# jctemp/owl-path-tracer

Hardware: AMD Instinct MI355X
Metric: Msamples/sec at 1920x1080x1024spp (higher is better)
Workload: dtype f32; 1 GPU; C4 dragon.json on the 871400-triangle stand-in (dragon.obj.scene is a missing blob), 1920x1080, 1024 spp, max_path_depth 16, environment intensity 0, areaLight emission 30; triangles=871404, bvh_nodes=276150, bvh_depth=24

## Files before the change

### owl-path-tracer_amd/csrc/pt_api.cpp

```cpp
#include <hip/hip_runtime.h>

#include <algorithm>
#include <atomic>
#include <chrono>
#include <cmath>
#include <cstdarg>
#include <cstdio>
#include <cstring>
#include <string>
#include <thread>
#include <vector>

#include "pt_internal.h"
#include "pt_launch.h"
#include "pt_tiers.h"

static inline void pt_collapse_sliver(float* p)
{
    const double e1[3] = {(double)p[3] - (double)p[0], (double)p[4] - (double)p[1], (double)p[5] - (double)p[2]};
    const double e2[3] = {(double)p[6] - (double)p[0], (double)p[7] - (double)p[1], (double)p[8] - (double)p[2]};
    const double e3[3] = {(double)p[6] - (double)p[3], (double)p[7] - (double)p[4], (double)p[8] - (double)p[5]};
    const double n[3] = {e1[1] * e2[2] - e1[2] * e2[1], e1[2] * e2[0] - e1[0] * e2[2], e1[0] * e2[1] - e1[1] * e2[0]};
    const double n2 = n[0] * n[0] + n[1] * n[1] + n[2] * n[2];
    const double l1 = e1[0] * e1[0] + e1[1] * e1[1] + e1[2] * e1[2], l2 = e2[0] * e2[0] + e2[1] * e2[1] + e2[2] * e2[2], l3 = e3[0] * e3[0] + e3[1] * e3[1] + e3[2] * e3[2];
    const double L2 = l1 > l2 ? (l1 > l3 ? l1 : l3) : (l2 > l3 ? l2 : l3);
    if (!(n2 > 1e-10 * L2 * L2)) {
        for (int k = 3; k < 9; ++k) p[k] = p[k % 3];
    }
}
#define PT_AUTO_PLOC_TRIS 64000000

namespace {
std::string g_create_error;
}

namespace pti {

int fail(pt_ctx* c, int code, const char* fmt, ...)
{
    char buf[1024];
    va_list ap;
    va_start(ap, fmt);
    vsnprintf(buf, sizeof(buf), fmt, ap);
    va_end(ap);
    if (c) c->err = buf;
    else g_create_error = buf;
    return code;
}

int ensure(pt_ctx* c, DevBuf& b, size_t bytes)
{
    if (bytes == 0) bytes = 16;
    if (b.cap >= bytes) return PT_OK;
    if (b.p) HIP_TRY(c, hipFree(b.p));
    b.p = nullptr;
    b.cap = 0;
    HIP_TRY(c, hipMalloc(&b.p, bytes));
    b.cap = bytes;
    return PT_OK;
}

}
using pti::ensure;
using pti::fail;

namespace {

int upload(pt_ctx* c, DevBuf& b, const void* src, size_t bytes)
{
    int rc = ensure(c, b, bytes);
    if (rc) return rc;
    if (bytes) HIP_TRY(c, hipMemcpyAsync(b.p, src, bytes, hipMemcpyHostToDevice, c->stream));
    return PT_OK;
}

void release(DevBuf& b)
{
    if (b.p) (void)hipFree(b.p);
    b.p = nullptr;
    b.cap = 0;
}

void copy_env(pt_ctx* c, const pt_env* env)
{
    c->env = *env;
    c->env_map.w = c->env_map.h = 0;
    c->env_map.px.clear();
    if (env->map.width > 0 && env->map.height > 0 && env->map.rgba8) {
        c->env_map.w = env->map.width;
        c->env_map.h = env->map.height;
        c->env_map.px.assign(env->map.rgba8, env->map.rgba8 + (size_t)env->map.width * env->map.height);
    }
    c->env.map.rgba8 = nullptr;
}

int upload_env(pt_ctx* c)
{
    if (c->host_only) return PT_OK;
    if (c->env_map.w > 0) return upload(c, c->d_env, c->env_map.px.data(), c->env_map.px.size() * 4);
    return PT_OK;
}

int upload_materials(pt_ctx* c)
{
    if (c->host_only) return PT_OK;
    return upload(c, c->d_materials, c->materials.data(), c->materials.size() * sizeof(float));
}

void pack_materials(pt_ctx* c, const float* materials, int n)
{
// ... 525 lines not shown

void walk_params(pt_ctx* c, const pt_camera* cam, PtKernelParams& P)
{
    fill_params(c, P);
    {
        const float reach = c->bvh.pad * 4194304.0f;
        float far_o = 0.0f;
        for (int a = 0; a < 3; ++a) far_o = std::max(far_o, std::fabs(cam->origin[a]));
        P.box_exact = (c->box_exact > 0 || (c->box_exact < 0 && !(far_o <= reach))) ? 1 : 0;
    }
    if (c->kernel == 2 && c->quad && !c->nodes4.empty()) {
        P.nodes4 = (const PtNode4*)c->d_nodes4.p;
        P.root = c->root4;
        P.stack_entries = 3 * c->depth4 + 1;
    }
    if (c->kernel == 2 && c->groups && !c->nodes8.empty()) {
        P.nodes8 = (const PtNode8*)c->d_nodes8.p;
        P.root8 = c->root8;
        P.groups = c->groups;
    }
}

struct FramePlan {
    int variant = 0, use_count = 0;
    PtGeometry geo{};
    int bpc = 0, grid = 0;
    int ring_grid = 0;
    bool sorted = false;
    bool tiers = false;
    int pre = 0;
    int n_launch = 1, S = 0;
    Schedule sc;
    int tail_min = 16;
    uint32_t n_express = 0;
    int express_waves = 0, ns_express = 0;
};

int plan_chunks(pt_ctx* c, bool group_walk, int max_samples, FramePlan& f)
{
    f.tail_min = c->chunk_tail_min >= 0 ? c->chunk_tail_min : 16;
    f.S = max_samples;
    f.n_launch = f.sorted ? 2 : 1;
    const int ns = f.geo.ns;
    if (f.sorted) {
        const int rest = max_samples - f.pre;
        int sticky = c->sticky_pct;
        if (sticky < 1) {
            const double ratio = (double)c->n_pixels / ((double)c->num_cus * (double)f.bpc * (double)ns);
            sticky = (int)std::min(80.0, 50.0 + 6.0 * ratio);
        }
        if (c->chunk_tail_min < 0) f.tail_min = std::max(16, rest / 8);
        const int big = std::max(1, (int)((int64_t)rest * sticky / 100));
        f.sc = make_schedule(rest, big, rest - big, f.tail_min);
    } else {
        const int chunk = std::min(c->spp_per_launch > 0 ? c->spp_per_launch : c->chunk_spp, std::min(max_samples, 65535));
        f.sc = make_schedule(max_samples, chunk, 1, f.tail_min);
    }
    const int n_chunks = f.sc.n_chunks;
    if ((uint64_t)c->n_pixels * (uint64_t)n_chunks >= 0xfff00000ull) return fail(c, PT_E_LIMIT, "too many (pixel, chunk) tickets");
    if (n_chunks > 255 || c->n_pixels >= (1u << 24)) return fail(c, PT_E_LIMIT, "the wavefront kernel needs n_chunks <= 255 and < 2^24 pixels per rank (raise chunk_spp)");
    if (f.sorted && group_walk && n_chunks <= 254 && (uint64_t)c->n_pixels * (uint64_t)n_chunks < 0xE0000000ull) {
        int& rgrid = f.tiers ? f.ring_grid : f.grid;
        const double ratio = (double)c->n_pixels / ((double)rgrid * (double)ns);
        double permille = c->express_permille >= 0 ? (double)c->express_permille : (ratio <= 1.5 ? 10.0 : (ratio >= 4.0 ? 0.0 : 10.0 * (4.0 - ratio) / 2.5));
        const int nse = std::max(1, std::min(c->ns_express, ns));
        uint64_t want = (uint64_t)((double)c->n_pixels * permille / 1000.0);
        const int capacity = c->num_cus * f.bpc;
        const int cap_waves = std::max(rgrid / 8, std::min(capacity / 2, capacity - rgrid));
        want = std::min<uint64_t>(want, (uint64_t)cap_waves * (uint64_t)nse);
        if (want > 0 && want < c->n_pixels) {
            f.n_express = (uint32_t)want;
            f.express_waves = (int)((want + (uint64_t)nse - 1) / (uint64_t)nse);
            f.ns_express = nse;
            rgrid = std::min(capacity, (int)(((long)c->n_pixels - (long)f.n_express + ns - 1) / ns) + f.express_waves);
        }
    }
    return PT_OK;
}

int plan_frame(pt_ctx* c, const PtKernelParams& P, int max_samples, FramePlan& f)
{
    f.use_count = (c->count || (c->kernel == 2 && !P.nodes4)) ? 1 : 0;
    f.variant = c->kernel == 2 && c->fallback && !f.use_count ? 3 : c->kernel;
    const int group_entries = P.nodes8 ? 7 * c->depth8 + 1 : 0;
    int want_ns = c->slots_per_wave > 0 ? c->slots_per_wave : PT_DEFAULT_NS;
    const PtGeometry& g = f.geo;
    auto geometry = [&] { return pt_kernel_geometry(f.variant, f.use_count, P.stack_entries, group_entries, want_ns, P.box_exact, &f.geo); };
    hipError_t ge = geometry();
    if (ge == hipErrorInvalidConfiguration && f.variant == 2 && !f.use_count) {
        f.variant = 3;
        ge = geometry();
    }
    if (ge == hipErrorInvalidConfiguration)
        return fail(c, PT_E_LIMIT, f.use_count ? "the instrumented instance of the render kernel needs scratch in this build; such builds rendered wrong pixels and are refused (pt_kernel.hip; tests/test_abi_host.py reads hipcc's resource report)"
                                               : "this build of the render kernel spills registers to scratch even in its fallback instance; such builds rendered wrong pixels and are refused (pt_kernel.hip)");
    HIP_TRY(c, ge);
    if (c->kernel == 2 && c->slots_per_wave == 0 && g.max_blocks_per_cu > 0) {
        const long fit = (long)c->n_pixels / ((long)c->num_cus * 8);
        if (fit < want_ns) {
            want_ns = (int)std::max(64L, fit);
            HIP_TRY(c, geometry());
        }
    }
    if (g.max_blocks_per_cu < 1) return fail(c, PT_E_LIMIT, "render kernel does not fit a CU (LDS %zu bytes, BVH depth %d)", g.lds_bytes, c->bvh.depth);
    f.bpc = c->blocks_per_cu > 0 ? std::min(c->blocks_per_cu, g.max_blocks_per_cu) : g.max_blocks_per_cu;
    const long capacity = (long)c->num_cus * f.bpc;
    const int per_wg = c->kernel == 1 ? g.block : g.ns;
    f.grid = (int)std::max(1L, std::min(((long)c->n_pixels + per_wg - 1) / per_wg, capacity));
    f.pre = c->prepass_spp > 0 ? c->prepass_spp : 8;
    f.sorted = c->kernel == 2 && c->schedule == 1 && c->spp_per_launch == 0 && max_samples >= 4 * f.pre && max_samples <= 65535;
    if (f.sorted && P.nodes8 && c->whole != 0 && c->slots_per_wave == 0) {
        for (int nsd = 96; nsd <= 104 && !f.tiers; nsd += 8) {
            if (c->whole < 1 && (long)c->n_pixels + (long)PT_MAX_TIERS * nsd > capacity * nsd) continue;
            want_ns = nsd;
            HIP_TRY(c, geometry());
            if (g.max_blocks_per_cu >= f.bpc && g.ns == nsd) {
                f.tiers = true;
                f.ring_grid = (int)std::max(1L, std::min(((long)c->n_pixels + g.ns - 1) / g.ns, capacity));
                f.grid = (int)capacity;
            }
        }
        if (!f.tiers) {
            want_ns = PT_DEFAULT_NS;
            HIP_TRY(c, geometry());
        }
    }
    if (f.tiers && c->prepass_spp == 0 && max_samples >= 4 * 16) f.pre = 16;
    if (c->kernel == 1) {
        f.S = std::min(c->spp_per_launch > 0 ? std::min(c->spp_per_launch, max_samples) : max_samples, 65535);
        f.n_launch = (max_samples + f.S - 1) / f.S;
        return PT_OK;
    }
    return plan_chunks(c, P.nodes8 != nullptr, max_samples, f);
}

int frame_buffers(pt_ctx* c, const FramePlan& f, int W, int H, void* d_out_rgb, void* d_out_rgba8, hipStream_t stream)
{
    int rc;
    const int n_chunks = f.sc.n_chunks;
    if (f.geo.state_words && (rc = ensure(c, c->d_slots, f.geo.state_words * 4 * (size_t)f.grid))) return rc;
    if (f.sorted) {
        if ((rc = ensure(c, c->d_cost, (size_t)W * H))) return rc;
        if ((rc = ensure(c, c->d_bucket, (size_t)c->n_pixels))) return rc;
        HIP_TRY(c, hipMemsetAsync(c->d_cost.p, 0, (size_t)W * H, stream));
        if ((rc = ensure(c, c->d_sorted, (size_t)c->n_pixels * 4))) return rc;
        if ((rc = ensure(c, c->d_sort_scratch, pt_sort_scratch_bytes(c->n_pixels)))) return rc;
    }
    if (c->kernel == 2) {
        c->lap_ticks_ofs = ((256 + (size_t)(n_chunks + 3) * 4 + 255) / 256) * 256;
        const size_t laps_bytes = c->lap_ticks_ofs + ((size_t)PT_LAP_REGION(n_chunks) + (size_t)PT_LAP_REGION(1)) * 8;
        if ((rc = ensure(c, c->d_laps, laps_bytes))) return rc;
        if ((rc = ensure(c, c->d_ring, (size_t)c->n_pixels * 4 * (size_t)n_chunks))) return rc;
        HIP_TRY(c, hipMemsetAsync(c->d_laps.p, 0, laps_bytes, stream));
        if (n_chunks > 1) HIP_TRY(c, hipMemsetAsync(c->d_ring.p, 0, (size_t)c->n_pixels * 4 * (size_t)n_chunks, stream));
        if ((rc = ensure(c, c->d_params, sizeof(PtKernelParams) * (size_t)f.n_launch))) return rc;
    }
    c->last_chunks = n_chunks;
    if ((rc = ensure(c, c->d_heads, (size_t)f.n_launch * PT_HEADS_WORDS * 4))) return rc;
    HIP_TRY(c, hipMemsetAsync(c->d_heads.p, 0, (size_t)f.n_launch * PT_HEADS_WORDS * 4, stream));
    if (f.tiers && (rc = ensure(c, c->d_tiers, (1 + PT_MAX_TIERS * PT_TIER_WORDS) * 4))) return rc;
    HIP_TRY(c, hipMemsetAsync(d_out_rgb, 0, (size_t)W * H * 3 * sizeof(float), stream));
    if (d_out_rgba8) HIP_TRY(c, hipMemsetAsync(d_out_rgba8, 0, (size_t)W * H * 4, stream));
    if (f.n_launch > 1 || n_chunks > 1) {
        if ((rc = ensure(c, c->d_rng, (size_t)W * H * 4))) return rc;
        if ((rc = ensure(c, c->d_accum, (size_t)W * H * 12))) return rc;
    }
// ... 185 lines not shown
    if (!c || !out) return PT_E_INVALID;
    if (!c->host_only && c->ev_pending) {
        HIP_TRY(c, hipSetDevice(c->device));
        HIP_TRY(c, hipEventSynchronize(c->ev1));
        int wrc = check_watchdog(c);
        if (wrc) return wrc;
        float ms = 0.0f;
        HIP_TRY(c, hipEventElapsedTime(&ms, c->ev0, c->ev1));
        c->stats.kernel_ms = ms;
        c->stats.prepass_ms = 0.0;
        if (c->last_sorted) {
            HIP_TRY(c, hipEventElapsedTime(&ms, c->ev0, c->evm));
            c->stats.prepass_ms = ms;
        }
        c->stats.launches = c->last_launches;
        c->ev_pending = false;
        if (c->count && c->d_counters.p) {
            PtCounters h;
            HIP_TRY(c, hipMemcpy(&h, c->d_counters.p, sizeof(h), hipMemcpyDeviceToHost));
            c->stats.samples = h.samples; c->stats.rays = h.rays; c->stats.nodes = h.nodes; c->stats.tris = h.tris;
            c->stats.scatters = h.scatters; c->stats.env_misses = h.env_misses; c->stats.nan_retries = h.nan_retries;
            for (int i = 0; i < 32; ++i) c->stats.sched[i] = h.sched[i];
            for (int i = 0; i < 8; ++i) c->stats.groups[i] = h.grp[i];
            for (int i = 0; i < 16; ++i) c->stats.lobes[i] = h.lobes[i];
            for (int i = 0; i < 4; ++i) c->stats.trav[i] = h.trav[i];
        }
    }
    *out = c->stats;
    return PT_OK;
}

void pt_to_camera_data(const float look_from[3], const float look_at[3], const float look_up[3], float vfov, int32_t w, int32_t h, pt_camera* out)
{
    auto dot = [](const float* a, const float* b) { return std::fma(a[2], b[2], std::fma(a[1], b[1], a[0] * b[0])); };
    auto cross = [](const float* a, const float* b, float* r) {
        r[0] = std::fma(a[1], b[2], -(a[2] * b[1]));
        r[1] = std::fma(a[2], b[0], -(a[0] * b[2]));
        r[2] = std::fma(a[0], b[1], -(a[1] * b[0]));
    };
    auto normalize = [&](float* v) {
        float s = 1.0f / std::sqrt(dot(v, v));
        v[0] *= s; v[1] *= s; v[2] *= s;
    };
    const float pi = 3.14159265358979323f;
    float aspect = (float)w / (float)h;
    float theta = vfov * pi / 180.0f;
    float hh = std::tan(theta / 2);
    float vh = 2.0f * hh, vw = aspect * vh;
    float W[3] = {look_from[0] - look_at[0], look_from[1] - look_at[1], look_from[2] - look_at[2]};
    normalize(W);
    float U[3], Vv[3];
    cross(look_up, W, U);
    normalize(U);
    cross(W, U, Vv);
    normalize(Vv);
    for (int i = 0; i < 3; ++i) {
        out->origin[i] = look_from[i];
        out->horizontal[i] = vw * U[i];
        out->vertical[i] = vh * Vv[i];
        out->llc[i] = look_from[i] - out->horizontal[i] / 2.0f - out->vertical[i] / 2.0f - W[i];
    }
}

int pt_debug_closest_hit_host(pt_ctx* c, const float org[3], const float dir[3], float tmin, float tmax, float* t, float* u, float* v, int32_t* prim)
{
    if (!c || !c->have_scene) return PT_E_NO_SCENE;
    return pt_bvh_closest_hit_host(c->bvh, org, dir, tmin, tmax, t, u, v, prim) ? 1 : 0;
}

int pt_debug_clone_scene(pt_ctx* dst, const pt_ctx* src)
{
    if (!dst || !src || dst == src) return PT_E_INVALID;
    return pti::clone_scene(dst, src);
}

int pt_debug_quad_info(pt_ctx* c, int64_t out[8])
{
    if (!c || !out) return PT_E_INVALID;
    if (!c->have_scene) return fail(c, PT_E_NO_SCENE, "pt_debug_quad_info before pt_upload_scene");
    int64_t leaf_slots = 0, tris = 0, empty = 0, internal = 0, bin_leaves = 0;
    for (const PtNode4& q : c->nodes4) {
        for (int k = 0; k < 4; ++k) {
            const int32_t r = q.child[k];
            if (r >= 0) ++internal;
            else if (r == -1) {
                ++empty;
                for (int a = 0; a < 3; ++a)
                    if (!(q.lo[a][k] == INFINITY && q.hi[a][k] == INFINITY)) return fail(c, PT_E_LIMIT, "quad node: empty slot with a finite box");
            } else {
                ++leaf_slots;
                tris += (int64_t)(~(uint32_t)r & 7u);
            }
        }
    }
    for (const PtNode& nd : c->bvh.nodes) {
        if (nd.left < -1) ++bin_leaves;
        if (nd.right < -1) ++bin_leaves;
    }
    out[0] = (int64_t)c->nodes4.size(); out[1] = c->depth4; out[2] = leaf_slots; out[3] = tris; out[4] = empty; out[5] = internal;
    out[6] = (int64_t)c->bvh.nodes.size(); out[7] = bin_leaves;
    return PT_OK;
}

int pt_debug_oct_info(pt_ctx* c, int64_t out[8])
{
    if (!c || !out) return PT_E_INVALID;
    if (!c->have_scene) return fail(c, PT_E_NO_SCENE, "pt_debug_oct_info before pt_upload_scene");
    int64_t leaf_slots = 0, tris = 0, empty = 0, internal = 0, max_leaf = 0;
    std::vector<uint8_t> seen(c->bvh.tris.size(), 0);
    std::vector<uint8_t> referenced(c->nodes8.size(), 0);
    for (const PtNode8& q : c->nodes8) {
        for (int k = 0; k < 8; ++k) {
            const int32_t r = q.c[k].ref;
            if (r >= 0) {
                if ((size_t)r >= c->nodes8.size() || referenced[(size_t)r]++) return fail(c, PT_E_LIMIT, "oct node: child %d out of range or referenced twice", r);
                ++internal;
            } else if (r == -1) {
                ++empty;
                for (int a = 0; a < 3; ++a)
                    if (!(q.c[k].lo[a] == INFINITY && q.c[k].hi[a] == INFINITY)) return fail(c, PT_E_LIMIT, "oct node: empty slot with a finite box");
            } else {
                const uint32_t code = ~(uint32_t)r, first = code >> 3, count = code & 7u;
                ++leaf_slots;
                tris += count;
                max_leaf = std::max<int64_t>(max_leaf, count);
                for (uint32_t t = first; t < first + count; ++t) {
                    if (t >= seen.size() || seen[t]++) return fail(c, PT_E_LIMIT, "oct node: triangle slot %u out of range or in two leaves", t);
                    const PtTri& tr = c->bvh.tris[t];
                    if (tr.id == 0x7fffffff) continue;
                    for (int a = 0; a < 3; ++a) {
                        const float lo = std::min(tr.p0[a], std::min(tr.p1[a], tr.p2[a])), hi = std::max(tr.p0[a], std::max(tr.p1[a], tr.p2[a]));
                        if (lo < q.c[k].lo[a] || hi > q.c[k].hi[a]) return fail(c, PT_E_LIMIT, "oct node: triangle slot %u sticks out of its leaf box", t);
                    }
                }
            }
        }
    }
    out[0] = (int64_t)c->nodes8.size(); out[1] = c->depth8; out[2] = leaf_slots; out[3] = tris; out[4] = empty; out[5] = internal;
    out[6] = max_leaf; out[7] = (int64_t)c->bvh.tris.size();
    return PT_OK;
}

int64_t pt_debug_read_queue(pt_ctx* c, uint32_t* queue_ids, uint32_t* input_ids, uint8_t* cost, int64_t cap)
{
    if (!c) return PT_E_INVALID;
    if (c->host_only) return fail(c, PT_E_NO_DEVICE, "host-only context: pt_debug_read_queue needs the GPU");
    if (!c->last_sorted) return 0;
    const int64_t n = std::min<int64_t>(cap, c->n_pixels);
    HIP_TRY(c, hipSetDevice(c->device));
    HIP_TRY(c, hipStreamSynchronize(c->stream));
    if (queue_ids) HIP_TRY(c, hipMemcpy(queue_ids, c->d_sorted.p, (size_t)n * 4, hipMemcpyDeviceToHost));
    if (input_ids) HIP_TRY(c, hipMemcpy(input_ids, c->d_pixels.p, (size_t)n * 4, hipMemcpyDeviceToHost));
    if (cost) {
        std::vector<uint8_t> img((size_t)c->last_w * (size_t)c->last_h);
        std::vector<uint32_t> ids((size_t)n);
        HIP_TRY(c, hipMemcpy(img.data(), c->d_cost.p, img.size(), hipMemcpyDeviceToHost));
        HIP_TRY(c, hipMemcpy(ids.data(), c->d_pixels.p, (size_t)n * 4, hipMemcpyDeviceToHost));
        for (int64_t i = 0; i < n; ++i) cost[i] = ids[(size_t)i] < img.size() ? img[ids[(size_t)i]] : 0;
    }
    return n;
}

int64_t pt_debug_read_laps(pt_ctx* c, uint64_t* ticks, int64_t cap)
{
    if (!c || !ticks) return PT_E_INVALID;
    if (c->host_only) return fail(c, PT_E_NO_DEVICE, "host-only context: pt_debug_read_laps needs the GPU");
    if (c->kernel != 2 || !c->d_laps.p) return 0;
    const int nt = 3 * (c->last_chunks + 1);
    std::vector<uint64_t> blk((size_t)PT_LAP_REGION(c->last_chunks));
    HIP_TRY(c, hipSetDevice(c->device));
    HIP_TRY(c, hipStreamSynchronize(c->stream));
    HIP_TRY(c, hipMemcpy(blk.data(), (char*)c->d_laps.p + c->lap_ticks_ofs, blk.size() * 8, hipMemcpyDeviceToHost));
    int64_t n = 0;
    for (int i = 0; i < nt && n < cap; ++i) ticks[n++] = blk[(size_t)i];
    for (int i = 0; i < 64 && n < cap; ++i) ticks[n++] = blk[(size_t)PT_LAP_DIAG_OFS(c->last_chunks) + i];
// ... 62 lines not shown
```

### owl-path-tracer_amd/csrc/pt_kernel.hip

```cpp
#include "pt_launch.h"
#include "pt_tiers.h"
#include "pt_trace.h"
#ifndef PT_WAVES_PER_EU
#define PT_WAVES_PER_EU 4
#endif
#ifndef PT_COUNT_WAVES_PER_EU
#define PT_COUNT_WAVES_PER_EU 2
#endif
#ifndef PT_WATCHDOG_ROUNDS
#define PT_WATCHDOG_ROUNDS 20000000
#endif
#ifndef PT_RAY_LOW
#define PT_RAY_LOW 32
#endif
#ifndef PT_MIN_BATCH
#define PT_MIN_BATCH 32
#endif
#ifndef PT_NODE_KEEP
#define PT_NODE_KEEP 24
#endif
#ifndef PT_NODE_BURSTS
#define PT_NODE_BURSTS 3
#endif
#ifndef PT_NODE_REPS
#define PT_NODE_REPS 2
#endif
#ifndef PT_QUAD_REPS
#define PT_QUAD_REPS 1
#endif
#ifndef PT_TOPUP_MIN
#define PT_TOPUP_MIN 8
#endif
#ifndef PT_ALLOW_SCRATCH
#define PT_ALLOW_SCRATCH 0
#endif
#ifndef PT_RETIRE_MIN
#define PT_RETIRE_MIN 16
#endif


namespace {

template <int STRIDE, int LDS_ENTRIES, bool CENSUS = false>
__device__ __forceinline__ void node4_step(const PtNode4* __restrict__ nodes4, uint32_t* stack, uint32_t PT_AS1* ovf, v3 o, v3 inv, float tbest, int& cur, int& sp,
                                           const bool exact, uint32_t* n_nohit = nullptr, uint32_t* n_beyond = nullptr)
{
    bool crossed = false;
    const size_t nb = (size_t)(uint32_t)cur * sizeof(PtNode4);
    const f32x4 lx = ldg4(nodes4, nb), ly = ldg4(nodes4, nb + 16), lz = ldg4(nodes4, nb + 32);
    const f32x4 hx = ldg4(nodes4, nb + 48), hy = ldg4(nodes4, nb + 64), hz = ldg4(nodes4, nb + 80), cf = ldg4(nodes4, nb + 96);
    const f32x2 ox = {o.x, o.x}, oy = {o.y, o.y}, oz = {o.z, o.z}, ix = {inv.x, inv.x}, iy = {inv.y, inv.y}, iz = {inv.z, inv.z};
    const float nx = -(o.x * inv.x), ny = -(o.y * inv.y), nz = -(o.z * inv.z);
    const f32x2 nox = {nx, nx}, noy = {ny, ny}, noz = {nz, nz};
    const f32x2 pad = {1.0000004f, 1.0000004f};
    float tn[4];
    bool hit[4];
#pragma unroll
    for (int p = 0; p < 2; ++p) {
        const f32x2 lox = p ? (f32x2){lx.z, lx.w} : (f32x2){lx.x, lx.y}, loy = p ? (f32x2){ly.z, ly.w} : (f32x2){ly.x, ly.y};
        const f32x2 loz = p ? (f32x2){lz.z, lz.w} : (f32x2){lz.x, lz.y}, hix = p ? (f32x2){hx.z, hx.w} : (f32x2){hx.x, hx.y};
        const f32x2 hiy = p ? (f32x2){hy.z, hy.w} : (f32x2){hy.x, hy.y}, hiz = p ? (f32x2){hz.z, hz.w} : (f32x2){hz.x, hz.y};
        f32x2 t0x, t1x, t0y, t1y, t0z, t1z;
        if (exact) {
            t0x = (lox - ox) * ix; t1x = (hix - ox) * ix;
            t0y = (loy - oy) * iy; t1y = (hiy - oy) * iy;
            t0z = (loz - oz) * iz; t1z = (hiz - oz) * iz;
        } else {
            t0x = __builtin_elementwise_fma(lox, ix, nox); t1x = __builtin_elementwise_fma(hix, ix, nox);
            t0y = __builtin_elementwise_fma(loy, iy, noy); t1y = __builtin_elementwise_fma(hiy, iy, noy);
            t0z = __builtin_elementwise_fma(loz, iz, noz); t1z = __builtin_elementwise_fma(hiz, iz, noz);
        }
        const float ta = fmax_hw(fmax_hw(fmin_hw(t0x.x, t1x.x), fmin_hw(t0y.x, t1y.x)), fmax_hw(fmin_hw(t0z.x, t1z.x), kTMin));
        const float tb = fmax_hw(fmax_hw(fmin_hw(t0x.y, t1x.y), fmin_hw(t0y.y, t1y.y)), fmax_hw(fmin_hw(t0z.y, t1z.y), kTMin));
        f32x2 tf = {fmin_hw(fmin_hw(fmax_hw(t0x.x, t1x.x), fmax_hw(t0y.x, t1y.x)), fmin_hw(fmax_hw(t0z.x, t1z.x), tbest)),
                    fmin_hw(fmin_hw(fmax_hw(t0x.y, t1x.y), fmax_hw(t0y.y, t1y.y)), fmin_hw(fmax_hw(t0z.y, t1z.y), tbest))};
        tf = tf * pad;
        tn[2 * p] = ta; tn[2 * p + 1] = tb;
        hit[2 * p] = ta <= tf.x; hit[2 * p + 1] = tb <= tf.y;
        if (CENSUS) {
            const float fa = fmin_hw(fmin_hw(fmax_hw(t0x.x, t1x.x), fmax_hw(t0y.x, t1y.x)), fmax_hw(t0z.x, t1z.x)) * 1.0000004f;
            const float fb = fmin_hw(fmin_hw(fmax_hw(t0x.y, t1x.y), fmax_hw(t0y.y, t1y.y)), fmax_hw(t0z.y, t1z.y)) * 1.0000004f;
            crossed = crossed || ta <= fa || tb <= fb;
        }
    }
    const int r0 = __float_as_int(cf.x), r1 = __float_as_int(cf.y), r2 = __float_as_int(cf.z), r3 = __float_as_int(cf.w);
    const float far_key = kTMax * 2.0f;
    const float k0 = hit[0] ? tn[0] : far_key, k1 = hit[1] ? tn[1] : far_key, k2 = hit[2] ? tn[2] : far_key, k3 = hit[3] ? tn[3] : far_key;
    const bool b01 = k1 < k0, b23 = k3 < k2;
    const float m01 = b01 ? k1 : k0, m23 = b23 ? k3 : k2;
    const int r01 = b01 ? r1 : r0, r23 = b23 ? r3 : r2;
    const bool in_b = m23 < m01;
    const int nearc = in_b ? r23 : r01;
    const bool any = hit[0] || hit[1] || hit[2] || hit[3];
    if (CENSUS) {
        *n_nohit += any ? 0u : 1u;
        *n_beyond += (!any && crossed) ? 1u : 0u;
    }
    const bool swap_o = in_b ? b01 : b23;
    const int oa = in_b ? r0 : r2, ob = in_b ? r1 : r3;
    const bool ha = in_b ? hit[0] : hit[2], hb = in_b ? hit[1] : hit[3];
    const int x1 = swap_o ? oa : ob, x2 = swap_o ? ob : oa;
    const bool h1 = swap_o ? ha : hb, h2 = swap_o ? hb : ha;
    const bool first_of_pair = in_b ? !b23 : !b01;
    const int x3 = in_b ? (first_of_pair ? r3 : r2) : (first_of_pair ? r1 : r0);
    const bool h3 = in_b ? (first_of_pair ? hit[3] : hit[2]) : (first_of_pair ? hit[1] : hit[0]);
    if (LDS_ENTRIES == 0x7fffffff) {
        stack[sp * STRIDE] = (uint32_t)x1; sp += h1 ? 1 : 0;
        stack[sp * STRIDE] = (uint32_t)x2; sp += h2 ? 1 : 0;
        stack[sp * STRIDE] = (uint32_t)x3; sp += h3 ? 1 : 0;
    } else {
        if (h1) { stack_push<STRIDE, LDS_ENTRIES>(stack, ovf, sp, (uint32_t)x1); ++sp; }
        if (h2) { stack_push<STRIDE, LDS_ENTRIES>(stack, ovf, sp, (uint32_t)x2); ++sp; }
        if (h3) { stack_push<STRIDE, LDS_ENTRIES>(stack, ovf, sp, (uint32_t)x3); ++sp; }
    }
    if (any) {
        cur = nearc;
    } else if (sp > 0) {
        --sp;
        cur = (int)stack_pop<STRIDE, LDS_ENTRIES>(stack, ovf, sp);
    } else {
        cur = PT_DONE;
    }
}

__device__ __forceinline__ uint32_t ld_agent(const uint32_t* p) { return __hip_atomic_load(gp(p), __ATOMIC_RELAXED, __HIP_MEMORY_SCOPE_AGENT); }
__device__ __forceinline__ void st_agent(uint32_t* p, uint32_t v) { __hip_atomic_store(gp(p), v, __ATOMIC_RELAXED, __HIP_MEMORY_SCOPE_AGENT); }
__device__ __forceinline__ uint32_t take_agent(uint32_t* p) { return __hip_atomic_fetch_add(gp(p), 1u, __ATOMIC_RELAXED, __HIP_MEMORY_SCOPE_AGENT); }

#define PT_NO_TICKET 0xfffffffeu
struct WaveTier {
    uint32_t* counter;
    uint32_t q0, count;
    bool express;
};
#define PT_EXPRESS 0xE0000000u
#define PT_WHOLE 255u
__device__ __forceinline__ uint32_t take_ticket(const PtKernelParams& P, const WaveTier& tier)
{
    if (tier.counter != nullptr) {
        const uint32_t e = take_agent(tier.counter);
        return e < tier.count ? PT_EXPRESS | (tier.q0 + e) : PT_NO_TICKET;
    }
    if (!tier.express) {
        const uint32_t t = take_agent(P.queue_head);
        if (t < P.n_tickets) return t;
    }
    if (P.n_express) {
        const uint32_t e = take_agent(P.queue_head + 64);
        if (e < P.n_express) return PT_EXPRESS | e;
    }
    return PT_NO_TICKET;
}

__device__ __forceinline__ bool start_chunk(const PtKernelParams& P, uint32_t ticket, uint32_t& c, int& px, int& py, uint32_t& rng, v3& color)
{
    uint32_t pid;
    const uint32_t n_bulk = P.n_pixels - P.n_express;
    if ((ticket & 0xF0000000u) == PT_EXPRESS) {
        pid = gp(P.pixel_ids)[ticket & 0x0FFFFFFFu];
        c = PT_WHOLE;
    } else if (ticket < n_bulk) {
        pid = gp(P.pixel_ids)[P.n_express + ticket];
        c = 0;
    } else {
        const uint32_t e = ld_agent(P.ring + ticket);
        if (e == 0u) return false;
        pid = e - 1u;
        c = ticket / n_bulk;
    }
    if (P.timeline && c != PT_WHOLE && ticket % n_bulk == n_bulk - 1u) gp(P.lap_ticks)[(P.n_chunks + 1) + 1 + c] = wall_clock64();
    px = (int)(pid % (uint32_t)P.width);
    py = (int)(pid / (uint32_t)P.width);
    if (c == 0 && P.dbg_start) gp(P.dbg_start)[pid] = (uint32_t)wall_clock64();
    if ((c == 0 || c == PT_WHOLE) && P.sample_begin == 0) {
        rng = rng_init((uint32_t)px, (uint32_t)py);
        color = vs(0.0f);
    } else {
        rng = ld_agent(P.rng_state + pid);
        const uint32_t* a = reinterpret_cast<const uint32_t*>(P.accum) + 3 * (size_t)pid;
        color = V(__uint_as_float(ld_agent(a)), __uint_as_float(ld_agent(a + 1)), __uint_as_float(ld_agent(a + 2)));
    }
    return true;
}

__device__ __forceinline__ int chunk_len(const PtKernelParams& P, uint32_t c)
{
    if (c == PT_WHOLE) return P.sample_count;
    return (int)c < P.n_full ? P.chunk_spp : P.tail_len[(int)c - P.n_full];
// ... 817 lines not shown
```

### owl-path-tracer_amd/csrc/pt_trace.h

```cpp
#pragma once
#include <cstdlib>

#include "pt_device.h"
#include "pt_types.h"

using namespace ptd;

#define PT_BLOCK 256
#define PT_DONE (-1)
#define PT_WAVE 64

namespace {

struct Hit {
    float t, u, v;
    int slot;
    int id;
};

struct Counters {
    uint32_t rays = 0, nodes = 0, tris = 0, scat = 0, env = 0, samples = 0, retry = 0;
    unsigned long long cyc[8] = {};
    uint32_t sched[32] = {};
    uint32_t depth[4] = {};
    uint32_t grp[6] = {};
    unsigned long long grp_cyc = 0;
    uint32_t lobe[16] = {};
    uint32_t cull_nohit = 0, cull_beyond = 0, leaf_noimp = 0;
};

#define PT_AS1 __attribute__((address_space(1)))
typedef float f32x4 __attribute__((ext_vector_type(4)));
template <class T>
__device__ __forceinline__ T PT_AS1* gp(T* p) { return (T PT_AS1*)p; }
__device__ __forceinline__ f32x4 ldg4(const void* base, size_t byte_off) { return *(const f32x4 PT_AS1*)((const char PT_AS1*)base + byte_off); }
__device__ __forceinline__ float fmin_hw(float a, float b) { return __builtin_fminf(a, b); }
__device__ __forceinline__ float fmax_hw(float a, float b) { return __builtin_fmaxf(a, b); }

__device__ __forceinline__ bool box_test(float bminx, float bminy, float bminz, float bmaxx, float bmaxy, float bmaxz, v3 o, v3 inv,
                                         float tbest, float& tnear)
{
    float t0x = (bminx - o.x) * inv.x, t1x = (bmaxx - o.x) * inv.x;
    float t0y = (bminy - o.y) * inv.y, t1y = (bmaxy - o.y) * inv.y;
    float t0z = (bminz - o.z) * inv.z, t1z = (bmaxz - o.z) * inv.z;
    float tn = fmax_hw(fmax_hw(fmin_hw(t0x, t1x), fmin_hw(t0y, t1y)), fmax_hw(fmin_hw(t0z, t1z), kTMin));
    float tf = fmin_hw(fmin_hw(fmax_hw(t0x, t1x), fmax_hw(t0y, t1y)), fmin_hw(fmax_hw(t0z, t1z), tbest));
    tnear = tn;
    return tn <= tf * 1.0000004f;
}

__device__ __forceinline__ bool box_test_fma(float bminx, float bminy, float bminz, float bmaxx, float bmaxy, float bmaxz, v3 o, v3 inv, float tbest, float& tnear)
{
    const float nx = -(o.x * inv.x), ny = -(o.y * inv.y), nz = -(o.z * inv.z);
    float t0x = fma_(bminx, inv.x, nx), t1x = fma_(bmaxx, inv.x, nx);
    float t0y = fma_(bminy, inv.y, ny), t1y = fma_(bmaxy, inv.y, ny);
    float t0z = fma_(bminz, inv.z, nz), t1z = fma_(bmaxz, inv.z, nz);
    float tn = fmax_hw(fmax_hw(fmin_hw(t0x, t1x), fmin_hw(t0y, t1y)), fmax_hw(fmin_hw(t0z, t1z), kTMin));
    float tf = fmin_hw(fmin_hw(fmax_hw(t0x, t1x), fmax_hw(t0y, t1y)), fmin_hw(fmax_hw(t0z, t1z), tbest));
    tnear = tn;
    return tn <= tf * 1.0000004f;
}

#ifndef PT_FAST_RAY_INV
#define PT_FAST_RAY_INV 1
#endif
#ifndef PT_INV_MAX
#define PT_INV_MAX 1e18f
#endif
__device__ __forceinline__ v3 ray_inv(v3 d)
{
#if PT_FAST_RAY_INV
    const float x = __builtin_amdgcn_rcpf(d.x), y = __builtin_amdgcn_rcpf(d.y), z = __builtin_amdgcn_rcpf(d.z);
#else
    const float x = 1.0f / d.x, y = 1.0f / d.y, z = 1.0f / d.z;
#endif
    return V(__builtin_amdgcn_fmed3f(x, -PT_INV_MAX, PT_INV_MAX), __builtin_amdgcn_fmed3f(y, -PT_INV_MAX, PT_INV_MAX), __builtin_amdgcn_fmed3f(z, -PT_INV_MAX, PT_INV_MAX));
}

__device__ __forceinline__ void tri_eval(const f32x4 a, const f32x4 b, const f32x4 c, int slot, v3 o, v3 d, Hit& h)
{
    v3 p0 = V(a.x, a.y, a.z), p1 = V(a.w, b.x, b.y), p2 = V(b.z, b.w, c.x);
    int id = __float_as_int(c.y);
    v3 e1 = p1 - p0, e2 = p2 - p0;
    v3 pv = cross(d, e2);
    float det = dot(e1, pv);
    float inv = 1.0f / det;
    v3 tv = o - p0;
    float u = dot(tv, pv) * inv;
    v3 qv = cross(tv, e1);
    float v = dot(d, qv) * inv;
    float t = dot(e2, qv) * inv;
    if (u >= 0.0f && v >= 0.0f && u + v <= 1.0f && t > kTMin && (t < h.t || (t == h.t && id < h.id))) {
        h.t = t; h.u = u; h.v = v; h.id = id; h.slot = slot;
    }
}
__device__ __forceinline__ void tri_test(const PtTri* __restrict__ tris, int slot, v3 o, v3 d, Hit& h)
{
    const size_t tb = (size_t)(uint32_t)slot * sizeof(PtTri);
    const f32x4 a = ldg4(tris, tb), b = ldg4(tris, tb + 16), c = ldg4(tris, tb + 32);
    tri_eval(a, b, c, slot, o, d, h);
}
#ifndef PT_LEAF_PREFETCH
#define PT_LEAF_PREFETCH 4
#endif
__device__ __forceinline__ void leaf_test(const PtTri* __restrict__ tris, int first, int count, v3 o, v3 d, Hit& h)
{
#if PT_LEAF_PREFETCH == 0
    for (int k = 0; k < count; ++k) tri_test(tris, first + k, o, d, h);
#else
    f32x4 ra[PT_LEAF_PREFETCH], rb[PT_LEAF_PREFETCH], rc[PT_LEAF_PREFETCH];
#pragma unroll
    for (int k = 0; k < PT_LEAF_PREFETCH; ++k) {
        const int kk = k < count ? k : count - 1;
        const size_t tb = (size_t)(uint32_t)(first + kk) * sizeof(PtTri);
        ra[k] = ldg4(tris, tb); rb[k] = ldg4(tris, tb + 16); rc[k] = ldg4(tris, tb + 32);
    }
#pragma unroll
    for (int k = 0; k < PT_LEAF_PREFETCH; ++k) {
        if (k < count) tri_eval(ra[k], rb[k], rc[k], first + k, o, d, h);
    }
    for (int k = PT_LEAF_PREFETCH; k < count; ++k) tri_test(tris, first + k, o, d, h);
#endif
}

template <int STRIDE, int LDS_ENTRIES>
__device__ __forceinline__ void stack_push(uint32_t* stack, uint32_t PT_AS1* ovf, int sp, uint32_t v)
{
    if (LDS_ENTRIES == 0x7fffffff || sp < LDS_ENTRIES) stack[sp * STRIDE] = v;
    else ovf[(sp - LDS_ENTRIES) * STRIDE] = v;
}
template <int STRIDE, int LDS_ENTRIES>
__device__ __forceinline__ uint32_t stack_pop(uint32_t* stack, uint32_t PT_AS1* ovf, int sp)
{
    if (LDS_ENTRIES == 0x7fffffff || sp < LDS_ENTRIES) return stack[sp * STRIDE];
    return ovf[(sp - LDS_ENTRIES) * STRIDE];
}

typedef float f32x2 __attribute__((ext_vector_type(2)));

template <int STRIDE, int LDS_ENTRIES>
__device__ __forceinline__ void node_step(const PtNode* __restrict__ nodes, uint32_t* stack, uint32_t PT_AS1* ovf, v3 o, v3 inv, float tbest, int& cur,
                                          int& sp, uint32_t* depth_census = nullptr)
{
    const size_t nb = (size_t)(uint32_t)cur * sizeof(PtNode);
    const f32x4 a = ldg4(nodes, nb), b = ldg4(nodes, nb + 16), c = ldg4(nodes, nb + 32), chf = ldg4(nodes, nb + 48);
    const int chl = __float_as_int(chf.x), chr = __float_as_int(chf.y);
    const f32x2 lox = {a.x, a.y}, loy = {a.z, a.w}, loz = {b.x, b.y}, hix = {b.z, b.w}, hiy = {c.x, c.y}, hiz = {c.z, c.w};
    const f32x2 ox = {o.x, o.x}, oy = {o.y, o.y}, oz = {o.z, o.z}, ix = {inv.x, inv.x}, iy = {inv.y, inv.y}, iz = {inv.z, inv.z};
    const f32x2 t0x = (lox - ox) * ix, t1x = (hix - ox) * ix;
    const f32x2 t0y = (loy - oy) * iy, t1y = (hiy - oy) * iy;
    const f32x2 t0z = (loz - oz) * iz, t1z = (hiz - oz) * iz;
    const float tl = fmax_hw(fmax_hw(fmin_hw(t0x.x, t1x.x), fmin_hw(t0y.x, t1y.x)), fmax_hw(fmin_hw(t0z.x, t1z.x), kTMin));
    const float tr = fmax_hw(fmax_hw(fmin_hw(t0x.y, t1x.y), fmin_hw(t0y.y, t1y.y)), fmax_hw(fmin_hw(t0z.y, t1z.y), kTMin));
    f32x2 tf = {fmin_hw(fmin_hw(fmax_hw(t0x.x, t1x.x), fmax_hw(t0y.x, t1y.x)), fmin_hw(fmax_hw(t0z.x, t1z.x), tbest)),
                fmin_hw(fmin_hw(fmax_hw(t0x.y, t1x.y), fmax_hw(t0y.y, t1y.y)), fmin_hw(fmax_hw(t0z.y, t1z.y), tbest))};
    const f32x2 pad = {1.0000004f, 1.0000004f};
    tf = tf * pad;
    const bool hl = tl <= tf.x, hr = tr <= tf.y;
    const bool right_first = hr && (!hl || tr < tl);
    const int nearc = right_first ? chr : chl;
    const int farc = right_first ? chl : chr;
    if (hl && hr) {
        stack_push<STRIDE, LDS_ENTRIES>(stack, ovf, sp, (uint32_t)farc);
        if (depth_census) { depth_census[0] += 1; depth_census[1] += sp >= 8; depth_census[2] += sp >= 12; depth_census[3] += sp >= 16; }
        ++sp;
    }
    if (hl || hr) {
        cur = nearc;
    } else if (sp > 0) {
        --sp;
        cur = (int)stack_pop<STRIDE, LDS_ENTRIES>(stack, ovf, sp);
    } else {
        cur = PT_DONE;
    }
}

template <bool COUNT>
__device__ __forceinline__ void closest_hit(const PtKernelParams& P, uint32_t* stack, v3 o, v3 d, Hit& h, Counters& cn)
{
    h.t = kTMax; h.u = 0.0f; h.v = 0.0f; h.id = 0x7fffffff; h.slot = -1;
    const v3 inv = V(1.0f / d.x, 1.0f / d.y, 1.0f / d.z);
    int sp = 0;
    int cur = P.root;
    const PtNode* __restrict__ nodes = P.nodes;
    const PtTri* __restrict__ tris = P.tris;
    for (;;) {
        while (cur >= 0) {
            if (COUNT) ++cn.nodes;
            node_step<PT_BLOCK, 0x7fffffff>(nodes, stack, nullptr, o, inv, h.t, cur, sp);
        }
        if (cur == PT_DONE) break;
        uint32_t code = ~(uint32_t)cur;
        int first = (int)(code >> 3), count = (int)(code & 7u);
        for (int i = 0; i < count; ++i) {
            if (COUNT) ++cn.tris;
            tri_test(tris, first + i, o, d, h);
        }
        if (sp == 0) break;
        --sp;
        cur = (int)stack[sp * PT_BLOCK];
    }
}

__device__ __forceinline__ v3 interp3(float bw, float bx, float by, v3 a, v3 b, v3 c)
{
    return V(fma_(by, c.x, fma_(bx, b.x, bw * a.x)), fma_(by, c.y, fma_(bx, b.y, bw * a.y)), fma_(by, c.z, fma_(bx, b.z, bw * a.z)));
}

struct PathState {
    uint32_t rng;
    v3 org, dir, throughput;
    int depth, lobe, retries;
};

enum { SR_CONTINUE = 0, SR_END = 1, SR_RETRY = 2 };

template <bool COUNT>
__device__ __forceinline__ int shade_hit(const PtKernelParams& P, const float* mats, int tslot, float hu, float hv, PathState& ps, v3& radiance,
                                         Counters& cn)
{
    radiance = vs(0.0f);
// ... 142 lines not shown
```

Baseline: 4431 Msamples/s.

## Use ray-sign near/far plane selection, integer sort keys, and paired triangle tests

The quad-node box test now picks the near and far slab planes per axis from the ray direction sign. That drops the per-slot min/max of t0/t1, and the node loads use 32-bit offsets. Child ordering sorts hit distances as unsigned integer keys with a miss sentinel, which simplifies the near/far child selection logic. Leaf triangle tests process triangles in pairs with packed two-wide FMA math and load only 40 bytes per triangle. Host-side checks are added for record sizes under 4 GiB and for finite node boxes, and degenerate slivers now collapse to a finite vertex. The cost is more address arithmetic per load and a dependence on inv sign bits being correct for zero directions.

```diff
diff --git a/owl-path-tracer_amd/csrc/pt_api.cpp b/owl-path-tracer_amd/csrc/pt_api.cpp
--- a/owl-path-tracer_amd/csrc/pt_api.cpp
+++ b/owl-path-tracer_amd/csrc/pt_api.cpp
@@ -25,7 +25,10 @@
     const double l1 = e1[0] * e1[0] + e1[1] * e1[1] + e1[2] * e1[2], l2 = e2[0] * e2[0] + e2[1] * e2[1] + e2[2] * e2[2], l3 = e3[0] * e3[0] + e3[1] * e3[1] + e3[2] * e3[2];
     const double L2 = l1 > l2 ? (l1 > l3 ? l1 : l3) : (l2 > l3 ? l2 : l3);
     if (!(n2 > 1e-10 * L2 * L2)) {
-        for (int k = 3; k < 9; ++k) p[k] = p[k % 3];
+        int f = 0;
+        while (f < 3 && !(std::isfinite(p[3 * f]) && std::isfinite(p[3 * f + 1]) && std::isfinite(p[3 * f + 2]))) ++f;
+        const float q[3] = {f < 3 ? p[3 * f] : 0.0f, f < 3 ? p[3 * f + 1] : 0.0f, f < 3 ? p[3 * f + 2] : 0.0f};
+        for (int k = 0; k < 9; ++k) p[k] = q[k % 3];
     }
 }
 #define PT_AUTO_PLOC_TRIS 64000000
@@ -717,6 +720,8 @@
 {
     f.use_count = (c->count || (c->kernel == 2 && !P.nodes4)) ? 1 : 0;
     f.variant = c->kernel == 2 && c->fallback && !f.use_count ? 3 : c->kernel;
+    if (c->kernel == 2 && (c->bvh.tris.size() * sizeof(PtTri) > 0xffffffffull || c->nodes4.size() * sizeof(PtNode4) > 0xffffffffull))
+        return fail(c, PT_E_LIMIT, "the wavefront kernel needs triangle records and quad nodes below 4 GiB each (%zu triangle slots, %zu quad nodes)", c->bvh.tris.size(), c->nodes4.size());
     const int group_entries = P.nodes8 ? 7 * c->depth8 + 1 : 0;
     int want_ns = c->slots_per_wave > 0 ? c->slots_per_wave : PT_DEFAULT_NS;
     const PtGeometry& g = f.geo;
@@ -1068,15 +1073,20 @@
     for (const PtNode4& q : c->nodes4) {
         for (int k = 0; k < 4; ++k) {
             const int32_t r = q.child[k];
-            if (r >= 0) ++internal;
-            else if (r == -1) {
+            if (r == -1) {
                 ++empty;
                 for (int a = 0; a < 3; ++a)
                     if (!(q.lo[a][k] == INFINITY && q.hi[a][k] == INFINITY)) return fail(c, PT_E_LIMIT, "quad node: empty slot with a finite box");
-            } else {
+                continue;
+            }
+            if (r >= 0) ++internal;
+            else {
                 ++leaf_slots;
                 tris += (int64_t)(~(uint32_t)r & 7u);
             }
+            for (int a = 0; a < 3; ++a)
+                if (!(std::isfinite(q.lo[a][k]) && std::isfinite(q.hi[a][k]) && q.lo[a][k] <= q.hi[a][k]))
+                    return fail(c, PT_E_LIMIT, "quad node: slot %d has a box that is not finite with lo <= hi on axis %d", k, a);
         }
     }
     for (const PtNode& nd : c->bvh.nodes) {
diff --git a/owl-path-tracer_amd/csrc/pt_kernel.hip b/owl-path-tracer_amd/csrc/pt_kernel.hip
--- a/owl-path-tracer_amd/csrc/pt_kernel.hip
+++ b/owl-path-tracer_amd/csrc/pt_kernel.hip
@@ -46,64 +46,59 @@
                                            const bool exact, uint32_t* n_nohit = nullptr, uint32_t* n_beyond = nullptr)
 {
     bool crossed = false;
-    const size_t nb = (size_t)(uint32_t)cur * sizeof(PtNode4);
-    const f32x4 lx = ldg4(nodes4, nb), ly = ldg4(nodes4, nb + 16), lz = ldg4(nodes4, nb + 32);
-    const f32x4 hx = ldg4(nodes4, nb + 48), hy = ldg4(nodes4, nb + 64), hz = ldg4(nodes4, nb + 80), cf = ldg4(nodes4, nb + 96);
+    const uint32_t ex = (uint32_t)(__float_as_int(inv.x) >> 31) & 48u;
+    const uint32_t ey = (uint32_t)(__float_as_int(inv.y) >> 31) & 48u;
+    const uint32_t ez = (uint32_t)(__float_as_int(inv.z) >> 31) & 48u;
+    const uint32_t rec = (uint32_t)cur * (uint32_t)sizeof(PtNode4);
+    const f32x4 nx4 = ldg4u(nodes4, rec + ex, 0), ny4 = ldg4u(nodes4, rec + ey, 16), nz4 = ldg4u(nodes4, rec + ez, 32);
+    const f32x4 fx4 = ldg4u(nodes4, rec + (ex ^ 48u), 0), fy4 = ldg4u(nodes4, rec + (ey ^ 48u), 16), fz4 = ldg4u(nodes4, rec + (ez ^ 48u), 32);
+    const f32x4 cf = ldg4u(nodes4, rec, 96);
     const f32x2 ox = {o.x, o.x}, oy = {o.y, o.y}, oz = {o.z, o.z}, ix = {inv.x, inv.x}, iy = {inv.y, inv.y}, iz = {inv.z, inv.z};
     const float nx = -(o.x * inv.x), ny = -(o.y * inv.y), nz = -(o.z * inv.z);
     const f32x2 nox = {nx, nx}, noy = {ny, ny}, noz = {nz, nz};
     const f32x2 pad = {1.0000004f, 1.0000004f};
-    float tn[4];
-    bool hit[4];
+    const uint32_t kMiss = 0xffffffffu;
+    uint32_t key[4];
 #pragma unroll
     for (int p = 0; p < 2; ++p) {
-        const f32x2 lox = p ? (f32x2){lx.z, lx.w} : (f32x2){lx.x, lx.y}, loy = p ? (f32x2){ly.z, ly.w} : (f32x2){ly.x, ly.y};
-        const f32x2 loz = p ? (f32x2){lz.z, lz.w} : (f32x2){lz.x, lz.y}, hix = p ? (f32x2){hx.z, hx.w} : (f32x2){hx.x, hx.y};
-        const f32x2 hiy = p ? (f32x2){hy.z, hy.w} : (f32x2){hy.x, hy.y}, hiz = p ? (f32x2){hz.z, hz.w} : (f32x2){hz.x, hz.y};
-        f32x2 t0x, t1x, t0y, t1y, t0z, t1z;
+        const f32x2 enx = p ? (f32x2){nx4.z, nx4.w} : (f32x2){nx4.x, nx4.y}, eny = p ? (f32x2){ny4.z, ny4.w} : (f32x2){ny4.x, ny4.y};
+        const f32x2 enz = p ? (f32x2){nz4.z, nz4.w} : (f32x2){nz4.x, nz4.y}, exx = p ? (f32x2){fx4.z, fx4.w} : (f32x2){fx4.x, fx4.y};
+        const f32x2 exy = p ? (f32x2){fy4.z, fy4.w} : (f32x2){fy4.x, fy4.y}, exz = p ? (f32x2){fz4.z, fz4.w} : (f32x2){fz4.x, fz4.y};
+        f32x2 tnx, tfx, tny, tfy, tnz, tfz;
         if (exact) {
-            t0x = (lox - ox) * ix; t1x = (hix - ox) * ix;
-            t0y = (loy - oy) * iy; t1y = (hiy - oy) * iy;
-            t0z = (loz - oz) * iz; t1z = (hiz - oz) * iz;
+            tnx = (enx - ox) * ix; tfx = (exx - ox) * ix;
+            tny = (eny - oy) * iy; tfy = (exy - oy) * iy;
+            tnz = (enz - oz) * iz; tfz = (exz - oz) * iz;
         } else {
-            t0x = __builtin_elementwise_fma(lox, ix, nox); t1x = __builtin_elementwise_fma(hix, ix, nox);
-            t0y = __builtin_elementwise_fma(loy, iy, noy); t1y = __builtin_elementwise_fma(hiy, iy, noy);
-            t0z = __builtin_elementwise_fma(loz, iz, noz); t1z = __builtin_elementwise_fma(hiz, iz, noz);
-        }
-        const float ta = fmax_hw(fmax_hw(fmin_hw(t0x.x, t1x.x), fmin_hw(t0y.x, t1y.x)), fmax_hw(fmin_hw(t0z.x, t1z.x), kTMin));
-        const float tb = fmax_hw(fmax_hw(fmin_hw(t0x.y, t1x.y), fmin_hw(t0y.y, t1y.y)), fmax_hw(fmin_hw(t0z.y, t1z.y), kTMin));
-        f32x2 tf = {fmin_hw(fmin_hw(fmax_hw(t0x.x, t1x.x), fmax_hw(t0y.x, t1y.x)), fmin_hw(fmax_hw(t0z.x, t1z.x), tbest)),
-                    fmin_hw(fmin_hw(fmax_hw(t0x.y, t1x.y), fmax_hw(t0y.y, t1y.y)), fmin_hw(fmax_hw(t0z.y, t1z.y), tbest))};
+            tnx = __builtin_elementwise_fma(enx, ix, nox); tfx = __builtin_elementwise_fma(exx, ix, nox);
+            tny = __builtin_elementwise_fma(eny, iy, noy); tfy = __builtin_elementwise_fma(exy, iy, noy);
+            tnz = __builtin_elementwise_fma(enz, iz, noz); tfz = __builtin_elementwise_fma(exz, iz, noz);
+        }
+        const float ta = fmax_hw(fmax_hw(tnx.x, tny.x), fmax_hw(tnz.x, kTMin));
+        const float tb = fmax_hw(fmax_hw(tnx.y, tny.y), fmax_hw(tnz.y, kTMin));
+        f32x2 tf = {fmin_hw(fmin_hw(tfx.x, tfy.x), fmin_hw(tfz.x, tbest)), fmin_hw(fmin_hw(tfx.y, tfy.y), fmin_hw(tfz.y, tbest))};
         tf = tf * pad;
-        tn[2 * p] = ta; tn[2 * p + 1] = tb;
-        hit[2 * p] = ta <= tf.x; hit[2 * p + 1] = tb <= tf.y;
+        key[2 * p] = ta <= tf.x ? __float_as_uint(ta) : kMiss;
+        key[2 * p + 1] = tb <= tf.y ? __float_as_uint(tb) : kMiss;
         if (CENSUS) {
-            const float fa = fmin_hw(fmin_hw(fmax_hw(t0x.x, t1x.x), fmax_hw(t0y.x, t1y.x)), fmax_hw(t0z.x, t1z.x)) * 1.0000004f;
-            const float fb = fmin_hw(fmin_hw(fmax_hw(t0x.y, t1x.y), fmax_hw(t0y.y, t1y.y)), fmax_hw(t0z.y, t1z.y)) * 1.0000004f;
+            const float fa = fmin_hw(fmin_hw(tfx.x, tfy.x), tfz.x) * 1.0000004f;
+            const float fb = fmin_hw(fmin_hw(tfx.y, tfy.y), tfz.y) * 1.0000004f;
             crossed = crossed || ta <= fa || tb <= fb;
         }
     }
     const int r0 = __float_as_int(cf.x), r1 = __float_as_int(cf.y), r2 = __float_as_int(cf.z), r3 = __float_as_int(cf.w);
-    const float far_key = kTMax * 2.0f;
-    const float k0 = hit[0] ? tn[0] : far_key, k1 = hit[1] ? tn[1] : far_key, k2 = hit[2] ? tn[2] : far_key, k3 = hit[3] ? tn[3] : far_key;
-    const bool b01 = k1 < k0, b23 = k3 < k2;
-    const float m01 = b01 ? k1 : k0, m23 = b23 ? k3 : k2;
-    const int r01 = b01 ? r1 : r0, r23 = b23 ? r3 : r2;
+    const bool b01 = key[1] < key[0], b23 = key[3] < key[2];
+    const uint32_t m01 = b01 ? key[1] : key[0], M01 = b01 ? key[0] : key[1], m23 = b23 ? key[3] : key[2], M23 = b23 ? key[2] : key[3];
+    const int n01 = b01 ? r1 : r0, f01 = b01 ? r0 : r1, n23 = b23 ? r3 : r2, f23 = b23 ? r2 : r3;
     const bool in_b = m23 < m01;
-    const int nearc = in_b ? r23 : r01;
-    const bool any = hit[0] || hit[1] || hit[2] || hit[3];
+    const int nearc = in_b ? n23 : n01;
+    const bool any = (in_b ? m23 : m01) != kMiss;
     if (CENSUS) {
         *n_nohit += any ? 0u : 1u;
         *n_beyond += (!any && crossed) ? 1u : 0u;
     }
-    const bool swap_o = in_b ? b01 : b23;
-    const int oa = in_b ? r0 : r2, ob = in_b ? r1 : r3;
-    const bool ha = in_b ? hit[0] : hit[2], hb = in_b ? hit[1] : hit[3];
-    const int x1 = swap_o ? oa : ob, x2 = swap_o ? ob : oa;
-    const bool h1 = swap_o ? ha : hb, h2 = swap_o ? hb : ha;
-    const bool first_of_pair = in_b ? !b23 : !b01;
-    const int x3 = in_b ? (first_of_pair ? r3 : r2) : (first_of_pair ? r1 : r0);
-    const bool h3 = in_b ? (first_of_pair ? hit[3] : hit[2]) : (first_of_pair ? hit[1] : hit[0]);
+    const int x1 = in_b ? f01 : f23, x2 = in_b ? n01 : n23, x3 = in_b ? f23 : f01;
+    const bool h1 = (in_b ? M01 : M23) != kMiss, h2 = (in_b ? m01 : m23) != kMiss, h3 = (in_b ? M23 : M01) != kMiss;
     if (LDS_ENTRIES == 0x7fffffff) {
         stack[sp * STRIDE] = (uint32_t)x1; sp += h1 ? 1 : 0;
         stack[sp * STRIDE] = (uint32_t)x2; sp += h2 ? 1 : 0;
diff --git a/owl-path-tracer_amd/csrc/pt_trace.h b/owl-path-tracer_amd/csrc/pt_trace.h
--- a/owl-path-tracer_amd/csrc/pt_trace.h
+++ b/owl-path-tracer_amd/csrc/pt_trace.h
@@ -34,6 +34,9 @@
 template <class T>
 __device__ __forceinline__ T PT_AS1* gp(T* p) { return (T PT_AS1*)p; }
 __device__ __forceinline__ f32x4 ldg4(const void* base, size_t byte_off) { return *(const f32x4 PT_AS1*)((const char PT_AS1*)base + byte_off); }
+__device__ __forceinline__ f32x4 ldg4u(const void* base, uint32_t byte_off, int imm) { return *(const f32x4 PT_AS1*)((const char PT_AS1*)base + (size_t)byte_off + imm); }
+typedef float f32x2 __attribute__((ext_vector_type(2)));
+__device__ __forceinline__ f32x2 ldg2u(const void* base, uint32_t byte_off, int imm) { return *(const f32x2 PT_AS1*)((const char PT_AS1*)base + (size_t)byte_off + imm); }
 __device__ __forceinline__ float fmin_hw(float a, float b) { return __builtin_fminf(a, b); }
 __device__ __forceinline__ float fmax_hw(float a, float b) { return __builtin_fmaxf(a, b); }
 
@@ -100,6 +103,33 @@
     const f32x4 a = ldg4(tris, tb), b = ldg4(tris, tb + 16), c = ldg4(tris, tb + 32);
     tri_eval(a, b, c, slot, o, d, h);
 }
+__device__ __forceinline__ void tri_take(float t, float u, float v, float uv, int id, int slot, Hit& h)
+{
+    if (u >= 0.0f && v >= 0.0f && uv <= 1.0f && t > kTMin && (t < h.t || (t == h.t && id < h.id))) {
+        h.t = t; h.u = u; h.v = v; h.id = id; h.slot = slot;
+    }
+}
+__device__ __forceinline__ f32x2 fma2(f32x2 a, f32x2 b, f32x2 c) { return __builtin_elementwise_fma(a, b, c); }
+__device__ __forceinline__ void tri_eval2(const f32x4 a0, const f32x4 b0, const f32x2 c0, const f32x4 a1, const f32x4 b1, const f32x2 c1, int slot0, bool take1,
+                                          const f32x2 ox, const f32x2 oy, const f32x2 oz, const f32x2 dx, const f32x2 dy, const f32x2 dz, Hit& h)
+{
+    const f32x2 p0x = {a0.x, a1.x}, p0y = {a0.y, a1.y}, p0z = {a0.z, a1.z};
+    const f32x2 p1x = {a0.w, a1.w}, p1y = {b0.x, b1.x}, p1z = {b0.y, b1.y};
+    const f32x2 p2x = {b0.z, b1.z}, p2y = {b0.w, b1.w}, p2z = {c0.x, c1.x};
+    const f32x2 e1x = p1x - p0x, e1y = p1y - p0y, e1z = p1z - p0z;
+    const f32x2 e2x = p2x - p0x, e2y = p2y - p0y, e2z = p2z - p0z;
+    const f32x2 pvx = fma2(dy, e2z, -(dz * e2y)), pvy = fma2(dz, e2x, -(dx * e2z)), pvz = fma2(dx, e2y, -(dy * e2x));
+    const f32x2 det = fma2(e1z, pvz, fma2(e1y, pvy, e1x * pvx));
+    const f32x2 inv = {1.0f / det.x, 1.0f / det.y};
+    const f32x2 tvx = ox - p0x, tvy = oy - p0y, tvz = oz - p0z;
+    const f32x2 u = fma2(tvz, pvz, fma2(tvy, pvy, tvx * pvx)) * inv;
+    const f32x2 qvx = fma2(tvy, e1z, -(tvz * e1y)), qvy = fma2(tvz, e1x, -(tvx * e1z)), qvz = fma2(tvx, e1y, -(tvy * e1x));
+    const f32x2 v = fma2(dz, qvz, fma2(dy, qvy, dx * qvx)) * inv;
+    const f32x2 t = fma2(e2z, qvz, fma2(e2y, qvy, e2x * qvx)) * inv;
+    const f32x2 uv = u + v;
+    tri_take(t.x, u.x, v.x, uv.x, __float_as_int(c0.y), slot0, h);
+    if (take1) tri_take(t.y, u.y, v.y, uv.y, __float_as_int(c1.y), slot0 + 1, h);
+}
 #ifndef PT_LEAF_PREFETCH
 #define PT_LEAF_PREFETCH 4
 #endif
@@ -108,18 +138,19 @@
 #if PT_LEAF_PREFETCH == 0
     for (int k = 0; k < count; ++k) tri_test(tris, first + k, o, d, h);
 #else
-    f32x4 ra[PT_LEAF_PREFETCH], rb[PT_LEAF_PREFETCH], rc[PT_LEAF_PREFETCH];
-#pragma unroll
-    for (int k = 0; k < PT_LEAF_PREFETCH; ++k) {
+    static_assert(PT_LEAF_PREFETCH == 4, "the leaf step tests the triangles of a leaf in two pairs");
+    f32x4 ra[4], rb[4];
+    f32x2 rc[4];
+#pragma unroll
+    for (int k = 0; k < 4; ++k) {
         const int kk = k < count ? k : count - 1;
-        const size_t tb = (size_t)(uint32_t)(first + kk) * sizeof(PtTri);
-        ra[k] = ldg4(tris, tb); rb[k] = ldg4(tris, tb + 16); rc[k] = ldg4(tris, tb + 32);
-    }
-#pragma unroll
-    for (int k = 0; k < PT_LEAF_PREFETCH; ++k) {
-        if (k < count) tri_eval(ra[k], rb[k], rc[k], first + k, o, d, h);
-    }
-    for (int k = PT_LEAF_PREFETCH; k < count; ++k) tri_test(tris, first + k, o, d, h);
+        const uint32_t tb = (uint32_t)(first + kk) * (uint32_t)sizeof(PtTri);
+        ra[k] = ldg4u(tris, tb, 0); rb[k] = ldg4u(tris, tb, 16); rc[k] = ldg2u(tris, tb, 32);
+    }
+    const f32x2 ox = {o.x, o.x}, oy = {o.y, o.y}, oz = {o.z, o.z}, dx = {d.x, d.x}, dy = {d.y, d.y}, dz = {d.z, d.z};
+    tri_eval2(ra[0], rb[0], rc[0], ra[1], rb[1], rc[1], first, count > 1, ox, oy, oz, dx, dy, dz, h);
+    if (count > 2) tri_eval2(ra[2], rb[2], rc[2], ra[3], rb[3], rc[3], first + 2, count > 3, ox, oy, oz, dx, dy, dz, h);
+    for (int k = 4; k < count; ++k) tri_test(tris, first + k, o, d, h);
 #endif
 }
 
@@ -135,8 +166,6 @@
     if (LDS_ENTRIES == 0x7fffffff || sp < LDS_ENTRIES) return stack[sp * STRIDE];
     return ovf[(sp - LDS_ENTRIES) * STRIDE];
 }
-
-typedef float f32x2 __attribute__((ext_vector_type(2)));
 
 template <int STRIDE, int LDS_ENTRIES>
 __device__ __forceinline__ void node_step(const PtNode* __restrict__ nodes, uint32_t* stack, uint32_t PT_AS1* ovf, v3 o, v3 inv, float tbest, int& cur,
```

After: 4836 Msamples/s, median of 6. 9.1% higher.
